# PereUbu7/Variational-Self-Organizing-Maps

Hardware: AMD Instinct MI355X
Metric: training samples/sec per epoch (BMU+update), 128x128 map, 784-dim (higher is better)
Workload: dtype f32

## Files before the change

variational-self-organizing-maps_amd/csrc/vsom_sl_i8.hip:

```cpp
#include "vsom_digits.hpp"
#include <cstdlib>

typedef int v4i __attribute__((ext_vector_type(4)));
typedef int v16i __attribute__((ext_vector_type(16)));
#ifdef VSOM_DEVELOPMENT
__device__ int vsom_sl_dbg = 0;
#endif

__device__ __forceinline__ void sl_kind_mark(unsigned *xflag, unsigned who)
{
    unsigned *slot = xflag + 32 * (1 + (who & 31u));
    if (__atomic_load_n(slot, __ATOMIC_RELAXED) == 0u)
        __atomic_store_n(slot, 1u, __ATOMIC_RELAXED);
}
__device__ __forceinline__ void sl_kind_fold(unsigned *xflag)
{
    const int lane = threadIdx.x & 63;
    const unsigned v = lane < 32 ? xflag[32 * (1 + lane)] : 0u;
    if (__ballot(v != 0u)) {
        if (lane < 32 && v != 0u)
            xflag[32 * (1 + lane)] = 0u;
        if (lane == 0)
            xflag[0] = 1u;
    }
}

__global__ __launch_bounds__(256) void sl_quant_rows_kernel(const float *__restrict__ src, int lds_, float *__restrict__ dst,
                                                            int ldd, const int *__restrict__ idx, int nrows,
                                                            signed char *__restrict__ xi, size_t xplane, int kp8,
                                                            float *__restrict__ lx, size_t lstride, unsigned *__restrict__ xflag)
{
    __shared__ float ssum[4], smax[4], sl1[4], snx[4];
    __shared__ int sa[4];
    const int row = blockIdx.x, lane = threadIdx.x & 63, wave = threadIdx.x >> 6;
    if (row >= nrows)
        return;
    const float *s = src + (size_t)row * lds_;
    auto value = [&](int k) -> float {
        if (k >= ldd)
            return 0.f;
        const int c = idx ? idx[k] : k;
        return c >= 0 ? s[c] : 0.f;
    };
    const int kend = xi ? kp8 : ldd;
    float sum = 0.f, mx = 0.f, l1f = 0.f, nx2 = 0.f;
    bool bad = false;
    float keep[4] = {0.f, 0.f, 0.f, 0.f};
    for (int k4 = threadIdx.x * 4; k4 < kend; k4 += 1024) {
        const float vv[4] = {value(k4), value(k4 + 1), value(k4 + 2), value(k4 + 3)};
#pragma unroll
        for (int u = 0; u < 4; ++u)
            keep[u] = vv[u];
        if (dst && k4 < ldd)
            *reinterpret_cast<float4 *>(dst + (size_t)row * ldd + k4) = make_float4(vv[0], vv[1], vv[2], vv[3]);
// ... 639 lines not shown
__device__ __forceinline__ void sl_gemm_i8_ring_body(const signed char *__restrict__ xi, size_t xplane, int s0, int s1,
                                                     const signed char *__restrict__ q, int N, int kp, int kp8,
                                                     const float *__restrict__ nrm, const double *__restrict__ qscale,
                                                     const double *__restrict__ qcorr, const float *__restrict__ xscale,
                                                     float *__restrict__ G, int ldg, float *__restrict__ tmin, int ntm,
                                                     signed char *ring, const int4 *__restrict__ qfast)
{
    constexpr int AUP = 4 * WM;
    constexpr int AU = AUP * XD;
    constexpr int UNITS = AU + 24;
    constexpr int UPW = UNITS / (2 * WM);
    constexpr int STAGE = UNITS * 1024, QOFF = AU * 1024, RTS = 64 * WM;
    static_assert(UNITS % (2 * WM) == 0 && NS * STAGE <= RING_BYTES, "ring layout");
    const int nchunks = (kp + IK - 1) / IK;
    const int tid = threadIdx.x, lane = tid & 63, wave = tid >> 6;
    const int wm = wave >> 1, wn = wave & 1;
    const int lr = lane & 31, lh = lane >> 5;
    const int sbase = s0 + blockIdx.y * RTS, nbase = blockIdx.x * RT_N;
    const size_t plane = (size_t)N * kp8;
    const signed char *xbase = XD == 1 ? xi : xi + xplane;

    unsigned soff[UPW];
    int dst[UPW];
#pragma unroll
    for (int i = 0; i < UPW; ++i) {
        const int id = wave * UPW + i;
        const int rin = lane >> 2, slot = lane & 3;
        if (id < AU) {
            const int pl = id / AUP, row = (id % AUP) * 16 + rin;
            int sr = sbase + row;
            sr = sr < s1 ? sr : s1 - 1;
            soff[i] = (unsigned)(pl * xplane + (size_t)sr * kp8 + ((slot ^ ((row >> 2) & 3)) << 4));
            dst[i] = id * 1024;
        } else {
            const int pl = (id - AU) >> 3, u = (id - AU) & 7;
            const int row = u * 16 + rin;
            int n = nbase + row;
            n = n < N ? n : N - 1;
            soff[i] = (unsigned)(pl * plane + (size_t)n * kp8 + ((slot ^ ((row >> 2) & 3)) << 4));
            dst[i] = QOFF + pl * 8192 + u * 1024;
        }
    }
    auto issue = [&](int c) {
        const int sb = (c % NS) * STAGE;
#pragma unroll
        for (int i = 0; i < UPW; ++i) {
            const signed char *base = (wave * UPW + i < AU ? xbase : q) + (size_t)c * IK;
            __builtin_amdgcn_global_load_lds((const __attribute__((address_space(1))) void *)(base + soff[i]),
                                             (__attribute__((address_space(3))) void *)(ring + sb + dst[i]), 16, 0, 0);
        }
    };

    v16i acc[3][2][2];
#pragma unroll
    for (int l = 0; l < 3; ++l)
#pragma unroll
        for (int i = 0; i < 2; ++i)
#pragma unroll
            for (int j = 0; j < 2; ++j)
#pragma unroll
                for (int r = 0; r < 16; ++r)
                    acc[l][i][j][r] = 0;

#pragma unroll
    for (int c = 0; c < NS - 1; ++c)
        if (c < nchunks)
            issue(c);
#ifdef VSOM_DEVELOPMENT
    const int dbg = vsom_sl_dbg;
#else
    constexpr int dbg = 0;
#endif
    for (int c = 0; c < ((dbg & 1) ? 1 : nchunks); ++c) {
        if (NS == 3 && c + 1 < nchunks)
            asm volatile("s_waitcnt vmcnt(%0)" ::"n"(UPW) : "memory");
        else
            asm volatile("s_waitcnt vmcnt(0)" ::: "memory");
        __syncthreads();
        if (c + NS - 1 < nchunks)
            issue(c + NS - 1);
        const signed char *st = ring + (c % NS) * STAGE;
#pragma unroll
        for (int ks = 0; ks < 2; ++ks) {
            v4i a[XD][2], b[3][2];
            const int P = ks * 2 + lh;
#pragma unroll
            for (int pl = 0; pl < XD; ++pl)
#pragma unroll
                for (int i = 0; i < 2; ++i) {
                    const int r = wm * 64 + i * 32 + lr;
                    a[pl][i] = *reinterpret_cast<const v4i *>(st + pl * (AUP * 1024) + r * 64 + ((P ^ ((r >> 2) & 3)) << 4));
                }
#pragma unroll
            for (int l = 0; l < 3; ++l)
#pragma unroll
                for (int j = 0; j < 2; ++j) {
                    const int r = wn * 64 + j * 32 + lr;
                    b[l][j] = *reinterpret_cast<const v4i *>(st + QOFF + l * 8192 + r * 64 + ((P ^ ((r >> 2) & 3)) << 4));
                }
#pragma unroll
            for (int pl = 0; pl < XD; ++pl)
#pragma unroll
                for (int l = 0; l + pl < 3; ++l)
#pragma unroll
                    for (int i = 0; i < 2; ++i)
#pragma unroll
                        for (int j = 0; j < 2; ++j)
                            acc[pl + l][i][j] = GLESS
                                                    ? __builtin_amdgcn_mfma_i32_32x32x32_i8(b[l][j], a[pl][i], acc[pl + l][i][j], 0, 0, 0)
                                                    : __builtin_amdgcn_mfma_i32_32x32x32_i8(a[pl][i], b[l][j], acc[pl + l][i][j], 0, 0, 0);
        }
    }
    if (dbg & 2)
        return;
    if (GLESS) {
        float *s_nrm = reinterpret_cast<float *>(ring);
        int4 *s_f = reinterpret_cast<int4 *>(ring + 512);
        __syncthreads();
        if (tid < RT_N) {
            const int n = nbase + tid;
            s_nrm[tid] = n < N ? nrm[n] : __uint_as_float(0x7F800000u);
            s_f[tid] = n < N ? qfast[n] : make_int4(0, 0, 0, 0);
        }
        float ts[2];
        int srow[2];
#pragma unroll
        for (int i = 0; i < 2; ++i) {
            srow[i] = sbase + wm * 64 + i * 32 + lr;
            ts[i] = XD == 3 ? xscale[srow[i] < s1 ? srow[i] : s1 - 1] : 1.f;
        }
        __syncthreads();
#pragma unroll
        for (int j = 0; j < 2; ++j) {
            const int nblk = nbase + wn * 64 + j * 32;
#pragma unroll
            for (int i = 0; i < 2; ++i) {
                float mn = __uint_as_float(0x7F800000u);
#pragma unroll
                for (int r = 0; r < 16; ++r) {
                    const int nl = wn * 64 + j * 32 + 4 * lh + (r & 3) + 8 * (r >> 2);
                    const float g = XD == 1 ? sl_i8_value_fast(acc[0][i][j][r], acc[1][i][j][r], acc[2][i][j][r], s_f[nl], s_nrm[nl])
                                            : sl_i8_value_fast3(acc[0][i][j][r], acc[1][i][j][r], acc[2][i][j][r], s_f[nl], ts[i], s_nrm[nl]);
                    mn = fminf(mn, g);
                }
                if (srow[i] < s1 && nblk < N)
                    tmin[(size_t)(srow[i] - s0) * ntm + (nblk >> 4) + lh] = mn;
            }
        }
        return;
    }
    const float inf = __uint_as_float(0x7F800000u);
    int col[2];
    double nm[2], sc[2], cr[2];
    int4 ff[2];
    float nmf[2];
#pragma unroll
    for (int j = 0; j < 2; ++j) {
        col[j] = nbase + wn * 64 + j * 32 + lr;
        const int cc = col[j] < N ? col[j] : N - 1;
        nmf[j] = nrm[cc];
        if (FAST) {
            ff[j] = qfast[cc];
        } else {
            nm[j] = (double)nmf[j];
            sc[j] = qscale[cc];
            cr[j] = XD == 1 ? qcorr[cc] : 0.0;
        }
    }
#pragma unroll
    for (int i = 0; i < 2; ++i) {
        float rsf[16];
        if (XD != 1) {
#pragma unroll
            for (int r = 0; r < 16; ++r) {
                const int row = sbase + wm * 64 + i * 32 + (r & 3) + 8 * (r >> 2) + 4 * lh;
                rsf[r] = xscale[row < s1 ? row : s1 - 1];
            }
        }
#pragma unroll
        for (int r = 0; r < 16; ++r) {
            float mn = inf;
#pragma unroll
            for (int j = 0; j < 2; ++j) {
                float g;
                if (FAST)
                    g = XD == 1 ? sl_i8_value_fast(acc[0][i][j][r], acc[1][i][j][r], acc[2][i][j][r], ff[j], nmf[j])
                                : sl_i8_value_fast3(acc[0][i][j][r], acc[1][i][j][r], acc[2][i][j][r], ff[j], rsf[r], nmf[j]);
                else
                    g = sl_i8_value(acc[0][i][j][r], acc[1][i][j][r], acc[2][i][j][r], cr[j],
                                    XD == 1 ? sc[j] : sc[j] * (double)rsf[r], nm[j]);
                acc[0][i][j][r] = __float_as_int(g);
                const float m = (col[j] < N && g == g) ? g : inf;
                mn = m < mn ? m : mn;
            }
            acc[1][i][0][r] = __float_as_int(sl_min32_dpp(mn));
        }
    }
    if (dbg & 4)
        return;
#pragma unroll
    for (int i = 0; i < 2; ++i) {
#pragma unroll
        for (int r = 0; r < 16; ++r) {
            const int row = sbase + wm * 64 + i * 32 + (r & 3) + 8 * (r >> 2) + 4 * lh;
            if (row < s1) {
                float *grow = G + (size_t)(row - s0) * ldg;
#pragma unroll
                for (int j = 0; j < 2; ++j)
                    if (col[j] < N)
                        grow[col[j]] = __int_as_float(acc[0][i][j][r]);
                if (lr == 31)
                    tmin[(size_t)(row - s0) * ntm + blockIdx.x * 2 + wn] = __int_as_float(acc[1][i][0][r]);
            }
        }
    }
}

__global__ __launch_bounds__(512, 1) void sl_gemm_i8_ring_kernel(const signed char *__restrict__ xi, size_t xplane, int s0, int s1,
                                                                 const signed char *__restrict__ q, int N, int kp,
                                                                 const unsigned *__restrict__ kp_dev, int kp8,
                                                                 const float *__restrict__ nrm, const double *__restrict__ qscale,
                                                                 const double *__restrict__ qcorr, const float *__restrict__ xscale,
                                                                 float *__restrict__ G, int ldg, float *__restrict__ tmin, int ntm,
                                                                 const unsigned *__restrict__ xflag,
                                                                 const int4 *__restrict__ qfast, unsigned *__restrict__ scal)
{
    if (kp_dev)
        kp = (int)kp_dev[2];
    if (blockIdx.x == 0 && blockIdx.y == 0 && threadIdx.x < 64)
        sl_fold_maxima(scal);
    extern __shared__ __attribute__((aligned(1024))) signed char ring[];
    if (xflag[0] != 0u) {
        if (qfast)
            sl_gemm_i8_ring_body<3, 4, 2, true>(xi, xplane, s0, s1, q, N, kp, kp8, nrm, qscale, qcorr, xscale, G, ldg, tmin, ntm, ring, qfast);
        else
            sl_gemm_i8_ring_body<3, 4, 2, false>(xi, xplane, s0, s1, q, N, kp, kp8, nrm, qscale, qcorr, xscale, G, ldg, tmin, ntm, ring, qfast);
    } else if (qfast)
        sl_gemm_i8_ring_body<1, 4, 3, true>(xi, xplane, s0, s1, q, N, kp, kp8, nrm, qscale, qcorr, xscale, G, ldg, tmin, ntm, ring, qfast);
    else
        sl_gemm_i8_ring_body<1, 4, 3, false>(xi, xplane, s0, s1, q, N, kp, kp8, nrm, qscale, qcorr, xscale, G, ldg, tmin, ntm, ring, qfast);
}

__global__ __launch_bounds__(512, 1) void sl_gemm_i8_ring_gless_kernel(const signed char *__restrict__ xi, size_t xplane, int s0, int s1,
                                                                       const signed char *__restrict__ q, int N, int kp,
                                                                       const unsigned *__restrict__ kp_dev, int kp8,
                                                                       const float *__restrict__ nrm, const float *__restrict__ xscale,
                                                                       float *__restrict__ tmin, int ntl,
                                                                       const unsigned *__restrict__ xflag,
                                                                       const int4 *__restrict__ qfast, unsigned *__restrict__ scal)
{
    if (kp_dev)
        kp = (int)kp_dev[2];
    if (blockIdx.x == 0 && blockIdx.y == 0 && threadIdx.x < 64)
        sl_fold_maxima(scal);
    extern __shared__ __attribute__((aligned(1024))) signed char ring[];
    if (xflag[0] != 0u)
        sl_gemm_i8_ring_body<3, 4, 2, true, true>(xi, xplane, s0, s1, q, N, kp, kp8, nrm, nullptr, nullptr, xscale, nullptr, 0, tmin, ntl, ring, qfast);
    else
        sl_gemm_i8_ring_body<1, 4, 3, true, true>(xi, xplane, s0, s1, q, N, kp, kp8, nrm, nullptr, nullptr, xscale, nullptr, 0, tmin, ntl, ring, qfast);
}

#define K64_NB 16
#define K64_SB 2
template <int XD>
__device__ __forceinline__ void sl_k64_body(const signed char *__restrict__ xi, size_t xplane, int s0, int s1,
                                            const signed char *__restrict__ q, int N, const float *__restrict__ xscale,
                                            float *__restrict__ tmin, int ntl, const float *s_nrm, const int4 *s_f)
{
    const int lane = threadIdx.x & 63, wave = threadIdx.x >> 6;
    const int lr = lane & 31, lh = lane >> 5;
    const int nbase = blockIdx.x * (K64_NB * 32);
    const size_t plane = (size_t)N * 64;
    v4i a[K64_SB][XD][2];
    float ts[K64_SB];
    bool sok[K64_SB];
    float *out[K64_SB];
#pragma unroll
    for (int sb = 0; sb < K64_SB; ++sb) {
        const int srow = s0 + (blockIdx.y * 4 + wave) * (32 * K64_SB) + sb * 32 + lr;
        sok[sb] = srow < s1;
        const size_t sr = (size_t)(sok[sb] ? srow : s1 - 1);
        const signed char *xbase = (XD == 1 ? xi : xi + xplane) + sr * 64 + 16 * lh;
#pragma unroll
        for (int pl = 0; pl < XD; ++pl)
#pragma unroll
            for (int ks = 0; ks < 2; ++ks)
                a[sb][pl][ks] = *reinterpret_cast<const v4i *>(xbase + pl * xplane + ks * 32);
        ts[sb] = XD == 3 ? xscale[sr] : 1.f;
        out[sb] = tmin + (size_t)(srow - s0) * ntl + (nbase >> 4) + lh;
    }
    const int nbn = (N - nbase + 31) / 32 < K64_NB ? (N - nbase + 31) / 32 : K64_NB;
    for (int nb = 0; nb < nbn; ++nb) {
        int n = nbase + nb * 32 + lr;
        n = n < N ? n : N - 1;
        const signed char *qb = q + (size_t)n * 64 + 16 * lh;
        v4i b[3][2];
#pragma unroll
        for (int l = 0; l < 3; ++l)
#pragma unroll
            for (int ks = 0; ks < 2; ++ks)
                b[l][ks] = *reinterpret_cast<const v4i *>(qb + l * plane + ks * 32);
        float nm[16], fx[16];
#pragma unroll
        for (int r = 0; r < 16; ++r) {
            const int nl = nb * 32 + 4 * lh + (r & 3) + 8 * (r >> 2);
            nm[r] = s_nrm[nl];
            fx[r] = __int_as_float(s_f[nl].x);
        }
#pragma unroll
        for (int sb = 0; sb < K64_SB; ++sb) {
            const v16i zero = {0, 0, 0, 0, 0, 0, 0, 0, 0, 0, 0, 0, 0, 0, 0, 0};
            v16i acc[3];
// ... 41 lines not shown
        s_nrm[i] = n < N ? nrm[n] : __uint_as_float(0x7F800000u);
        s_f[i] = n < N ? qfast[n] : make_int4(0, 0, 0, 0);
    }
    if (blockIdx.x == 0 && blockIdx.y == 0 && threadIdx.x < 64)
        sl_fold_maxima(scal);
    __syncthreads();
    if (xflag[0] != 0u)
        sl_k64_body<3>(xi, xplane, s0, s1, q, N, xscale, tmin, ntl, s_nrm, s_f);
    else
        sl_k64_body<1>(xi, xplane, s0, s1, q, N, xscale, tmin, ntl, s_nrm, s_f);
}

static int sl_i8_ensure(vsom_ctx *c, uint32_t kp8)
{
    const bool rekey = !c->sl_q.p || c->sl_kp8 != kp8;
    if (rekey) {
        VSOM_ALLOC_CHECK(vsom_grow_set(c->stream, VSOM_BUF_SYNC | VSOM_BUF_REBUILD,
                                     {vsom_member(c->sl_q, (size_t)3 * c->N * kp8), vsom_member(c->sl_qscale, c->N),
                                      vsom_member(c->sl_qcorr, c->N), vsom_member(c->sl_qfast, c->N)}));
        c->sl_kp8 = kp8;
    }
    if (rekey || (size_t)4 * c->Bcap * kp8 > c->sl_xi.cap) {
        VSOM_ALLOC_CHECK(vsom_grow_set(c->stream, VSOM_BUF_SYNC | VSOM_BUF_REBUILD,
                                     {vsom_member(c->sl_xi, (size_t)4 * c->Bcap * kp8), vsom_member(c->sl_l1, (size_t)5 * c->Bcap)}));
        c->xi_valid = false;
    }
    return VSOM_OK;
}

int launch_sl_gather_quant(vsom_ctx *c, size_t B, hipStream_t stream, const int *idx, bool *xi_out)
{
    const uint32_t kp8 = (c->cpitch + 63) / 64 * 64;
    const bool xi = c->sl_xi.p && c->sl_kp8 == kp8 && (size_t)4 * c->Bcap * kp8 <= c->sl_xi.cap && c->sl_scal.p;
    if (kp8 == 64)
        hipLaunchKernelGGL(sl_quant_rows64_kernel, dim3((unsigned)((B + 15) / 16)), dim3(256), 0, stream, c->Xs.p, (int)c->xpitch, c->Xc.p,
                           (int)c->cpitch, idx, (int)B, xi ? c->sl_xi.p : (signed char *)nullptr, (size_t)c->Bcap * kp8,
                           xi ? c->sl_l1.p : (float *)nullptr, (size_t)c->Bcap, xi ? c->sl_scal.p + 8192 : (unsigned *)nullptr);
    else
    hipLaunchKernelGGL(sl_quant_rows_kernel, dim3((unsigned)B), dim3(256), 0, stream, c->Xs.p, (int)c->xpitch, c->Xc.p,
                       (int)c->cpitch, idx, (int)B, xi ? c->sl_xi.p : (signed char *)nullptr, (size_t)c->Bcap * kp8, (int)kp8,
                       xi ? c->sl_l1.p : (float *)nullptr, (size_t)c->Bcap, xi ? c->sl_scal.p + 8192 : (unsigned *)nullptr);
    VSOM_HIP_CHECK(hipGetLastError());
    *xi_out = xi;
    return VSOM_OK;
}

int sl_i8_plan(vsom_ctx *c, size_t s0, size_t s1)
{
    const uint32_t kp8 = ((c->cc_valid ? c->cpitch : c->xpitch) + 63) / 64 * 64;
    if (kp8 == 64)
        return 1;
    const size_t big_tiles = ((size_t)c->N + RT_N - 1) / RT_N * ((s1 - s0 + RT_S - 1) / RT_S);
    if (kp8 <= 960 && big_tiles >= 256) {
        if (hipFuncSetAttribute((const void *)sl_gemm_i8_ring_gless_kernel, hipFuncAttributeMaxDynamicSharedMemorySize,
                                RING_BYTES) == hipSuccess)
            return 2;
        (void)hipGetLastError();
    }
    return 0;
}

int launch_sl_i8(vsom_ctx *c, size_t s0, size_t s1, size_t ldg, size_t ntm, unsigned *scal, unsigned *xflag, int plan)
{
    const bool gless = plan == 1;
    const bool compact = c->cc_valid;
    const uint32_t kmax = compact ? c->cpitch : c->xpitch;
    const uint32_t kp8 = (kmax + 63) / 64 * 64;
    if (int rc = sl_i8_ensure(c, kp8))
        return rc;
#ifdef VSOM_DEVELOPMENT
    {
        static int last = -1;
        const char *e = std::getenv("VSOM_SL_DBG");
        const int v = e ? std::atoi(e) : 0;
        if (v != last) {
            (void)hipMemcpyToSymbol(HIP_SYMBOL(vsom_sl_dbg), &v, sizeof(int));
            last = v;
        }
    }
#endif
    const size_t xplane = (size_t)c->Bcap * kp8;
    if (!c->xi_valid) {
        if (kp8 == 64)
            hipLaunchKernelGGL(sl_quant_rows64_kernel, dim3((unsigned)((c->B + 15) / 16)), dim3(256), 0, c->stream,
                               compact ? c->Xc.p : c->Xs.p, (int)kmax, (float *)nullptr, (int)kmax, (const int *)nullptr, (int)c->B,
                               c->sl_xi.p, xplane, c->sl_l1.p, (size_t)c->Bcap, xflag);
        else
        hipLaunchKernelGGL(sl_quant_rows_kernel, dim3((unsigned)c->B), dim3(256), 0, c->stream, compact ? c->Xc.p : c->Xs.p, (int)kmax,
                           (float *)nullptr, (int)kmax, (const int *)nullptr, (int)c->B, c->sl_xi.p, xplane, (int)kp8, c->sl_l1.p,
                           (size_t)c->Bcap, xflag);
        c->xi_valid = true;
    }
    const float *xscale = c->sl_l1.p + c->Bcap;
    const unsigned *kp_dev = compact ? (const unsigned *)c->cc_meta.p : nullptr;
    if (kp8 == 64 && c->part_pitch <= 64)
        hipLaunchKernelGGL(sl_prepare64_kernel, dim3((unsigned)((c->N + 15) / 16)), dim3(256), 0, c->stream, c->map.p, (int)c->pitch,
                           (int)c->part_pitch, (int)c->N, compact ? (const int *)c->cc_idx.p : (const int *)nullptr, (int)kmax, kp_dev,
                           c->sl_q.p, c->sl_nrm.p, c->sl_qscale.p, c->sl_qcorr.p, c->sl_qfast.p, scal, xflag);
    else
    hipLaunchKernelGGL(sl_prepare_i8_kernel, dim3((unsigned)((c->N + 3) / 4)), dim3(256), 0, c->stream, c->map.p, (int)c->pitch,
                       (int)c->part_pitch, (int)c->N, compact ? (const int *)c->cc_idx.p : (const int *)nullptr, (int)kmax, kp_dev,
                       (int)kp8, c->sl_q.p, c->sl_nrm.p, c->sl_qscale.p, c->sl_qcorr.p, c->sl_qfast.p, scal, xflag);
    const int4 *qfast = kp8 <= 960 ? c->sl_qfast.p : (const int4 *)nullptr;
    if (gless) {
        if (kp8 != 64)
            return VSOM_ERR_INVALID;
        dim3 grid((unsigned)((c->N + K64_NB * 32 - 1) / (K64_NB * 32)), (unsigned)((s1 - s0 + 128 * K64_SB - 1) / (128 * K64_SB)));
        hipLaunchKernelGGL(sl_k64_kernel, grid, dim3(256), 0, c->stream, c->sl_xi.p, xplane, (int)s0, (int)s1, c->sl_q.p, (int)c->N,
                           c->sl_nrm.p, c->sl_qfast.p, xscale, c->sl_tmin.p, (int)ntm, (const unsigned *)xflag, scal);
        VSOM_HIP_CHECK(hipGetLastError());
        return VSOM_OK;
    }
    if (plan == 2) {
        dim3 grid((unsigned)((c->N + RT_N - 1) / RT_N), (unsigned)((s1 - s0 + RT_S - 1) / RT_S));
        hipLaunchKernelGGL(sl_gemm_i8_ring_gless_kernel, grid, dim3(512), RING_BYTES, c->stream, c->sl_xi.p, xplane, (int)s0, (int)s1,
                           c->sl_q.p, (int)c->N, (int)kmax, kp_dev, (int)kp8, c->sl_nrm.p, xscale, c->sl_tmin.p, (int)ntm,
                           (const unsigned *)xflag, c->sl_qfast.p, scal);
        VSOM_HIP_CHECK(hipGetLastError());
        return VSOM_OK;
    }
    const size_t big_tiles = ((size_t)c->N + RT_N - 1) / RT_N * ((s1 - s0 + RT_S - 1) / RT_S);
    bool ring_ok = false;
    if (big_tiles >= 1024) {
        ring_ok = hipFuncSetAttribute((const void *)sl_gemm_i8_ring_kernel, hipFuncAttributeMaxDynamicSharedMemorySize,
                                      RING_BYTES) == hipSuccess;
        if (!ring_ok)
            (void)hipGetLastError();
    }
    if (ring_ok) {
        dim3 grid((unsigned)(ntm / 2), (unsigned)((s1 - s0 + RT_S - 1) / RT_S));
        hipLaunchKernelGGL(sl_gemm_i8_ring_kernel, grid, dim3(512), RING_BYTES, c->stream, c->sl_xi.p, xplane, (int)s0, (int)s1,
                           c->sl_q.p, (int)c->N, (int)kmax, kp_dev, (int)kp8, c->sl_nrm.p, c->sl_qscale.p, c->sl_qcorr.p, xscale, c->sl_G.p,
                           (int)ldg, c->sl_tmin.p, (int)ntm, (const unsigned *)xflag, qfast, scal);
    } else {
        constexpr int MI = 2;
        dim3 grid((unsigned)ntm, (unsigned)((s1 - s0 + 64 * MI - 1) / (64 * MI)));
        hipLaunchKernelGGL((sl_gemm_i8_kernel<MI, 1>), grid, dim3(256), 0, c->stream, c->sl_xi.p, xplane, (int)s0, (int)s1, c->sl_q.p,
                           (int)c->N, (int)kmax, kp_dev, (int)kp8, c->sl_nrm.p, c->sl_qscale.p, c->sl_qcorr.p, xscale, c->sl_G.p, (int)ldg,
                           c->sl_tmin.p, (int)ntm, (const unsigned *)xflag, qfast, scal);
        hipLaunchKernelGGL((sl_gemm_i8_kernel<MI, 3>), grid, dim3(256), 0, c->stream, c->sl_xi.p, xplane, (int)s0, (int)s1, c->sl_q.p,
                           (int)c->N, (int)kmax, kp_dev, (int)kp8, c->sl_nrm.p, c->sl_qscale.p, c->sl_qcorr.p, xscale, c->sl_G.p, (int)ldg,
                           c->sl_tmin.p, (int)ntm, (const unsigned *)xflag, qfast, scal);
    }
    VSOM_HIP_CHECK(hipGetLastError());
    return VSOM_OK;
}
```

variational-self-organizing-maps_amd/csrc/vsom_update.hip:

```cpp
#include "vsom_device.hpp"
#include <algorithm>
#include <cmath>
#include <cstdlib>
#include <mutex>


#define CWP_WT 512
#define CWP_THREADS (64 + CWP_WT)
template <int NW, int T, bool LUT_LDS, bool CONLY>
__global__ __launch_bounds__(CWP_THREADS) void cwp_kernel(const u64 *__restrict__ lastbmu, int B, int n0, int n1,
                                                          int W, int H, const float *__restrict__ lut,
                                                          int lutw, int luth, float2 *__restrict__ cw, int ldn,
                                                          float *__restrict__ weight)
{
    static_assert(NW * T == 2048 && CWP_WT % NW == 0 && T % 4 == 0 && T <= CWP_WT, "worker mapping");
    constexpr int LK = NW * T / CWP_WT;
    constexpr int PK = LK / 2;
    constexpr int QK = LK / 4;
    static_assert(LK % 4 == 0, "whole sample quads per worker thread");
    constexpr int SS = CWP_WT / NW;
    extern __shared__ __attribute__((aligned(16))) unsigned char cwp_smem[];
    float *wL = (float *)cwp_smem;
    float *WL = wL + 3 * T * NW;
    int2 *bL = (int2 *)(WL + 2 * T * NW);
    float *slut = (float *)(bL + 3 * T);
    const int tid = threadIdx.x;
    if (LUT_LDS) {
        for (int i = tid; i < lutw * luth; i += CWP_THREADS)
            slut[i] = lut[i];
    }
    const float *tab = LUT_LDS ? slut : lut;
    const int ntiles = (B + T - 1) / T;
    const int nloc = n1 - n0;
    const int wt = tid - 64;
    const int lnode = (wt < 0 ? tid : wt) & (NW - 1);
    const int s0 = wt < 0 ? 0 : wt / NW;
    const int nl = blockIdx.x * NW + lnode;
    const bool valid = nl < nloc;
    int cx = 0, cy = 0;
    if (valid)
        vsom_somindex((u64)(n0 + nl), (u64)W, (u64)H, cx, cy);

    auto load_bxy = [&](int t) {
        if (t < ntiles && wt < T) {
            const int j = t * T + wt;
            int bx = 0, by = 0;
            if (j < B)
                vsom_somindex(lastbmu[j], (u64)W, (u64)H, bx, by);
            bL[(t % 3) * T + wt] = make_int2(bx, by);
        }
    };
    auto lookup = [&](int t) {
        float *dst = wL + (t % 3) * T * NW;
        const int2 *bsrc = bL + (t % 3) * T;
        const int nt = B - t * T < T ? B - t * T : T;
        int2 b[LK];
        float w[LK];
#pragma unroll
        for (int k = 0; k < LK; ++k)
            b[k] = bsrc[s0 + k * SS];
#pragma unroll
        for (int k = 0; k < LK; ++k) {
            int dx = cx - b[k].x, dy = cy - b[k].y;
            dx = dx < 0 ? -dx : dx;
            dy = dy < 0 ? -dy : dy;
            dx = dx < lutw ? dx : lutw - 1;
            dy = dy < luth ? dy : luth - 1;
            w[k] = tab[dy * lutw + dx];
        }
#pragma unroll
        for (int k = 0; k < LK; ++k)
            if (s0 + k * SS < nt)
                dst[(s0 + k * SS) * NW + lnode] = w[k];
    };
    auto emit = [&](int t) {
        const float *ws = wL + (t % 3) * T * NW;
        const float *Ws = WL + (t & 1) * T * NW;
        const int nt = B - t * T < T ? B - t * T : T;
        if (CONLY) {
            float w[QK][4], Wp[QK][4];
#pragma unroll
            for (int k = 0; k < QK; ++k) {
                const int s = (s0 + k * SS) * 4;
#pragma unroll
                for (int i = 0; i < 4; ++i) {
                    w[k][i] = ws[(s + i) * NW + lnode];
                    Wp[k][i] = Ws[(s + i) * NW + lnode];
                }
            }
#pragma unroll
            for (int k = 0; k < QK; ++k) {
                const int s = (s0 + k * SS) * 4;
                float4 o;
                o.x = w[k][0] / Wp[k][0];
                o.y = s + 1 < nt ? w[k][1] / Wp[k][1] : 0.f;
                o.z = s + 2 < nt ? w[k][2] / Wp[k][2] : 0.f;
                o.w = s + 3 < nt ? w[k][3] / Wp[k][3] : 0.f;
                if (valid && s < nt)
                    ((float4 *)cw)[(size_t)((t * T + s) >> 2) * ldn + nl] = o;
            }
            return;
        }
        float w0[PK], w1[PK], W0[PK], W1[PK];
#pragma unroll
        for (int k = 0; k < PK; ++k) {
            const int s = (s0 + k * SS) * 2;
            w0[k] = ws[s * NW + lnode];
            W0[k] = Ws[s * NW + lnode];
            w1[k] = ws[(s + 1) * NW + lnode];
            W1[k] = Ws[(s + 1) * NW + lnode];
        }
#pragma unroll
        for (int k = 0; k < PK; ++k) {
            const int s = (s0 + k * SS) * 2;
            float4 o;
            o.x = w0[k] / W0[k];
            o.y = w0[k];
            const bool two = s + 1 < nt;
            o.z = two ? w1[k] / W1[k] : 0.f;
            o.w = two ? w1[k] : 0.f;
            if (valid && s < nt)
                ((float4 *)cw)[(size_t)((t * T + s) >> 1) * ldn + nl] = o;
        }
    };

    float run = 0.f;
    if (wt >= 0) {
        load_bxy(0);
        load_bxy(1);
    }
    __syncthreads();
    if (wt >= 0)
        lookup(0);
    __syncthreads();
    for (int t = 0; t < ntiles; ++t) {
        if (wt >= 0) {
            load_bxy(t + 2);
            if (t + 1 < ntiles)
                lookup(t + 1);
            if (t > 0)
                emit(t - 1);
        } else {
            const float *ws = wL + (t % 3) * T * NW;
            float *Ws = WL + (t & 1) * T * NW;
            const int nt = B - t * T < T ? B - t * T : T;
            int s = 0;
            for (; s + 16 <= nt; s += 16) {
                float r[16], o[16];
#pragma unroll
                for (int k = 0; k < 16; ++k)
                    r[k] = ws[(s + k) * NW + lnode];
#pragma unroll
                for (int k = 0; k < 16; ++k) {
                    run = run + r[k];
                    o[k] = run;
                }
                if (tid < NW) {
#pragma unroll
                    for (int k = 0; k < 16; ++k)
                        Ws[(s + k) * NW + lnode] = o[k];
                }
            }
            for (; s < nt; ++s) {
                run = run + ws[s * NW + lnode];
                if (tid < NW)
                    Ws[s * NW + lnode] = run;
            }
        }
        __syncthreads();
    }
    if (wt >= 0)
        emit(ntiles - 1);
    else if (tid < NW && valid && weight)
        weight[n0 + nl] = run;
}

typedef float vsom_f2 __attribute__((ext_vector_type(2)));

#define VSOM_MED_STEP(XS, CW)                                                                    \
    "v_pk_fma_f32 %[t], %[M], %[k24], " XS " neg_lo:[0,1,0] neg_hi:[0,1,0]\n\t"                   \
    "v_pk_mul_f32 %[p], %[t], %[k127] clamp\n\t"                                                  \
    "v_pk_mul_f32 %[n], %[t], %[k127] neg_lo:[1,0] neg_hi:[1,0] clamp\n\t"                        \
    "v_pk_fma_f32 %[M], " CW ", %[p], %[M] op_sel_hi:[0,1,1]\n\t"                                 \
    "v_pk_fma_f32 %[S], " CW ", %[p], %[S] op_sel:[1,0,0]\n\t"                                    \
    "v_pk_fma_f32 %[M], " CW ", %[n], %[M] op_sel_hi:[0,1,1] neg_lo:[1,0,0] neg_hi:[1,0,0]\n\t"   \
    "v_pk_fma_f32 %[S], " CW ", %[n], %[S] op_sel:[1,0,0]\n\t"

__device__ __forceinline__ void vsom_median_steps8(vsom_f2 &M, vsom_f2 &S, const vsom_f2 (&xs)[8], const float4 (&cv)[4])
{
    const vsom_f2 k24 = {0x1.0p24f, 0x1.0p24f}, k127 = {0x1.0p127f, 0x1.0p127f};
    const vsom_f2 c0 = {cv[0].x, cv[0].y}, c1 = {cv[0].z, cv[0].w}, c2 = {cv[1].x, cv[1].y}, c3 = {cv[1].z, cv[1].w},
                  c4 = {cv[2].x, cv[2].y}, c5 = {cv[2].z, cv[2].w}, c6 = {cv[3].x, cv[3].y}, c7 = {cv[3].z, cv[3].w};
    vsom_f2 t, p, n;
    asm volatile(VSOM_MED_STEP("%[x0]", "%[c0]") VSOM_MED_STEP("%[x1]", "%[c1]") VSOM_MED_STEP("%[x2]", "%[c2]")
                 VSOM_MED_STEP("%[x3]", "%[c3]") VSOM_MED_STEP("%[x4]", "%[c4]") VSOM_MED_STEP("%[x5]", "%[c5]")
                 VSOM_MED_STEP("%[x6]", "%[c6]") VSOM_MED_STEP("%[x7]", "%[c7]")
                 : [M] "+v"(M), [S] "+v"(S), [t] "=&v"(t), [p] "=&v"(p), [n] "=&v"(n)
                 : [x0] "v"(xs[0]), [x1] "v"(xs[1]), [x2] "v"(xs[2]), [x3] "v"(xs[3]), [x4] "v"(xs[4]), [x5] "v"(xs[5]),
                   [x6] "v"(xs[6]), [x7] "v"(xs[7]), [c0] "v"(c0), [c1] "v"(c1), [c2] "v"(c2), [c3] "v"(c3), [c4] "v"(c4),
                   [c5] "v"(c5), [c6] "v"(c6), [c7] "v"(c7), [k24] "s"(k24), [k127] "s"(k127));
}

__device__ __forceinline__ void vsom_median_step1(vsom_f2 &M, vsom_f2 &S, vsom_f2 xs, vsom_f2 cw)
{
    const vsom_f2 k24 = {0x1.0p24f, 0x1.0p24f}, k127 = {0x1.0p127f, 0x1.0p127f};
    vsom_f2 t, p, n;
    asm volatile(VSOM_MED_STEP("%[x0]", "%[c0]")
                 : [M] "+v"(M), [S] "+v"(S), [t] "=&v"(t), [p] "=&v"(p), [n] "=&v"(n)
                 : [x0] "v"(xs), [c0] "v"(cw), [k24] "s"(k24), [k127] "s"(k127));
}

template <bool MEDIAN, int FMA, int PLOG>
__global__ __launch_bounds__(256, 1) void update_chain3_kernel(const float *__restrict__ Xs, int ldx,
                                                               const float2 *__restrict__ cw, int ldn, int B,
                                                               int n0, int nloc, int D,
                                                               float *__restrict__ map,
                                                               float *__restrict__ sigma, int pitch,
                                                               const float *__restrict__ weight)
{
// ... 266 lines not shown
    if (need > c->lut.cap) {
        VSOM_HIP_CHECK(hipStreamSynchronize(c->stream));
        VSOM_ALLOC_CHECK(vsom_grow_set(c->stream, 0, {vsom_member(c->lut, need), vsom_member(c->lut_host, 2 * need)}));
        c->lut_ev_valid[0] = c->lut_ev_valid[1] = false;
    }
    const int k = c->lut_slot;
    c->lut_slot ^= 1;
    if (!c->lut_ev[k])
        VSOM_HIP_CHECK(hipEventCreateWithFlags(&c->lut_ev[k], hipEventDisableTiming));
    if (c->lut_ev_valid[k])
        VSOM_HIP_CHECK(hipEventSynchronize(c->lut_ev[k]));
    float *host = c->lut_host.p + (size_t)k * c->lut.cap;
    for (uint32_t dy = 0; dy < lh; ++dy)
        for (uint32_t dx = 0; dx < lw; ++dx)
            host[(size_t)dy * lw + dx] = (float)vsom_neighbourhood_weight(dx, dy, 0, 0, sigma);
    VSOM_HIP_CHECK(hipMemcpyAsync(c->lut.p, host, need * sizeof(float), hipMemcpyHostToDevice, c->stream));
    VSOM_HIP_CHECK(hipEventRecord(c->lut_ev[k], c->stream));
    c->lut_ev_valid[k] = true;
    c->lut_sigma = sigma;
    c->lut_w = lw;
    c->lut_h = lh;
    return VSOM_OK;
}

__global__ void empty_epoch_kernel(float *__restrict__ map, float *__restrict__ sigma, float *__restrict__ weight,
                                   int pitch, int part_pitch, int part_len, int n0, int nloc)
{
    const size_t i = (size_t)blockIdx.x * blockDim.x + threadIdx.x;
    if (i >= (size_t)nloc * pitch)
        return;
    const int nl = (int)(i / pitch), col = (int)(i % pitch);
    const size_t at = (size_t)(n0 + nl) * pitch + col;
    const float zero = weight[n0 + nl] * 0.f;
    map[at] = 0.f;
    sigma[at] = (col % part_pitch) < part_len ? sqrtf(0.f / (zero * 0.f + 0.f)) : 0.f;
}

__global__ void zero_weight_kernel(float *__restrict__ weight, int n0, int nloc)
{
    const int i = blockIdx.x * blockDim.x + threadIdx.x;
    if (i < nloc)
        weight[n0 + i] = 0.f;
}

static bool vsom_use_chain(const vsom_ctx *c, size_t nloc)
{
    if (!c->use_chain || c->transform == VSOM_CLR)
        return false;
    return ((nloc + 63) / 64) * ((c->D + 13) / 14) <= VSOM_CHAIN_MAX_WAVES;
}

extern "C" int vsom_small_map_chains(const vsom_ctx *c, size_t nodes) { return c && vsom_use_chain(c, nodes) ? 1 : 0; }

static int launch_cwp(vsom_ctx *c, const u64 *bmu, size_t B_, size_t n0, size_t n1, size_t ldn, bool conly, float *weight)
{
    const size_t nloc = n1 - n0;
    const size_t lut_bytes = (size_t)c->lut_w * c->lut_h * sizeof(float);
    const bool lds = lut_bytes <= 24 * 1024;
    constexpr int nw = 16, T = 2048 / nw;
    const size_t smem = (size_t)5 * 2048 * sizeof(float) + (size_t)3 * T * sizeof(int2) + (lds ? lut_bytes : 0);
    const void *fn = conly ? (lds ? (const void *)cwp_kernel<nw, T, true, true> : (const void *)cwp_kernel<nw, T, false, true>)
                           : (lds ? (const void *)cwp_kernel<nw, T, true, false> : (const void *)cwp_kernel<nw, T, false, false>);
    if (smem > 64 * 1024)
        VSOM_HIP_CHECK(hipFuncSetAttribute(fn, hipFuncAttributeMaxDynamicSharedMemorySize, (int)smem));
    int B = (int)B_, in0 = (int)n0, in1 = (int)n1, iW = (int)c->W, iH = (int)c->H, lw = (int)c->lut_w, lh = (int)c->lut_h,
        ildn = (int)ldn;
    const float *lut = c->lut.p;
    float2 *cwp = c->cw.p;
    void *args[] = {&bmu, &B, &in0, &in1, &iW, &iH, &lut, &lw, &lh, &cwp, &ildn, &weight};
    VSOM_HIP_CHECK(hipLaunchKernel(fn, dim3((unsigned)((nloc + nw - 1) / nw)), dim3(CWP_THREADS), args, smem, c->stream));
    return VSOM_OK;
}

static int launch_nt_chains(vsom_ctx *c, void *fn, size_t n0, size_t nloc, size_t B, size_t ldn, uint32_t bpad, bool compact,
                            const unsigned *meta, unsigned block = 512)
{
    const unsigned gx = (unsigned)((nloc + 63) / 64);
    const unsigned cols = compact ? c->cpitch : c->pitch;
    const unsigned quads = compact ? c->cpitch / 4 : (c->D + 3) / 4;
    UpdAsmArgs a;
    a.xs = c->Xq.p;
    a.cw2 = c->cw.p;
    a.map = compact ? c->Uc_map.p : c->map.p;
    a.sbuf = compact ? c->Uc_S.p : c->sigma.p;
    a.ldx_bytes = bpad * 16u;
    a.ldn_bytes = (unsigned)(ldn * 16u);
    a.B = (unsigned)B;
    a.nloc = (unsigned)nloc;
    a.nslices = quads;
    a.pitch_bytes = cols * 4u;
    a.n0 = (unsigned)n0;
    a.ppitch_bytes = 0;
    a.yp = compact ? (const void *)meta : nullptr;
    a.zq = c->zq.p;
    size_t sz = 80;
    void *extra[] = {HIP_LAUNCH_PARAM_BUFFER_POINTER, &a, HIP_LAUNCH_PARAM_BUFFER_SIZE, &sz, HIP_LAUNCH_PARAM_END};
    VSOM_HIP_CHECK(hipModuleLaunchKernel((hipFunction_t)fn, 8 * ((quads + 7) / 8), (gx + 7) / 8, 1, block, 1, 1, 0, c->stream,
                                         nullptr, extra));
    return VSOM_OK;
}

__global__ __launch_bounds__(256) void sg_keep_record_kernel(const int *__restrict__ inv, int ninv, const unsigned *__restrict__ meta,
                                                             int *__restrict__ inv_out, unsigned *__restrict__ meta_out,
                                                             const u64 *__restrict__ bmu, int nb, u64 *__restrict__ bmu_out)
{
    const int i = blockIdx.x * blockDim.x + threadIdx.x;
    if (i < ninv)
        inv_out[i] = inv[i];
    if (i < 16 && ninv > 0)
        meta_out[i] = meta[i];
    if (i < nb)
        bmu_out[i] = bmu[i];
}

void vsom_sigma_drop(vsom_ctx *c)
{
    if (c->sg.on) {
        c->sg.on = false;
        ++c->sg_stats[1];
    }
}

static int sigma_materialise(vsom_ctx *c)
// ... 191 lines not shown
```

Baseline: 1.793 million.

## Specialize gless GEMM by kind and tile size, retune cwp kernel with LDS row swizzle

Templatizes the gless ring GEMM kernel on the x-plane count and wave-M count. It adds a smaller 256-thread, two-blocks-per-CU variant for large grids and launches both kinds, each kernel returning early if the flag does not match. The first chunk's MFMAs now take a zero accumulator instead of an explicit zeroing pass, and the epilogue loads norms and fast coefficients from LDS as vectors. The cwp neighbourhood kernel gains a 112/448 worker configuration with an XOR row rotation meant to cut LDS bank conflicts on large c-only maps. These changes add an extra empty kernel launch and more template instantiations.

```diff
diff --git a/variational-self-organizing-maps_amd/csrc/vsom_sl_i8.hip b/variational-self-organizing-maps_amd/csrc/vsom_sl_i8.hip
--- a/variational-self-organizing-maps_amd/csrc/vsom_sl_i8.hip
+++ b/variational-self-organizing-maps_amd/csrc/vsom_sl_i8.hip
@@ -1,5 +1,6 @@
 #include "vsom_digits.hpp"
 #include <cstdlib>
+#include <type_traits>
 
 typedef int v4i __attribute__((ext_vector_type(4)));
 typedef int v16i __attribute__((ext_vector_type(16)));
@@ -745,15 +746,17 @@
     };
 
     v16i acc[3][2][2];
-#pragma unroll
-    for (int l = 0; l < 3; ++l)
-#pragma unroll
-        for (int i = 0; i < 2; ++i)
-#pragma unroll
-            for (int j = 0; j < 2; ++j)
-#pragma unroll
-                for (int r = 0; r < 16; ++r)
-                    acc[l][i][j][r] = 0;
+    if (!GLESS) {
+#pragma unroll
+        for (int l = 0; l < 3; ++l)
+#pragma unroll
+            for (int i = 0; i < 2; ++i)
+#pragma unroll
+                for (int j = 0; j < 2; ++j)
+#pragma unroll
+                    for (int r = 0; r < 16; ++r)
+                        acc[l][i][j][r] = 0;
+    }
 
 #pragma unroll
     for (int c = 0; c < NS - 1; ++c)
@@ -764,7 +767,8 @@
 #else
     constexpr int dbg = 0;
 #endif
-    for (int c = 0; c < ((dbg & 1) ? 1 : nchunks); ++c) {
+    auto chunk = [&](int c, auto open) {
+        constexpr bool OPEN = decltype(open)::value;
         if (NS == 3 && c + 1 < nchunks)
             asm volatile("s_waitcnt vmcnt(%0)" ::"n"(UPW) : "memory");
         else
@@ -798,11 +802,22 @@
 #pragma unroll
                     for (int i = 0; i < 2; ++i)
 #pragma unroll
-                        for (int j = 0; j < 2; ++j)
+                        for (int j = 0; j < 2; ++j) {
+                            const v16i zero = {0, 0, 0, 0, 0, 0, 0, 0, 0, 0, 0, 0, 0, 0, 0, 0};
+                            const v16i cin = (OPEN && ks == 0 && pl == 0) ? zero : acc[pl + l][i][j];
                             acc[pl + l][i][j] = GLESS
-                                                    ? __builtin_amdgcn_mfma_i32_32x32x32_i8(b[l][j], a[pl][i], acc[pl + l][i][j], 0, 0, 0)
-                                                    : __builtin_amdgcn_mfma_i32_32x32x32_i8(a[pl][i], b[l][j], acc[pl + l][i][j], 0, 0, 0);
-        }
+                                                    ? __builtin_amdgcn_mfma_i32_32x32x32_i8(b[l][j], a[pl][i], cin, 0, 0, 0)
+                                                    : __builtin_amdgcn_mfma_i32_32x32x32_i8(a[pl][i], b[l][j], cin, 0, 0, 0);
+                        }
+        }
+    };
+    if (GLESS) {
+        chunk(0, std::true_type());
+        for (int c = 1; c < ((dbg & 1) ? 1 : nchunks); ++c)
+            chunk(c, std::false_type());
+    } else {
+        for (int c = 0; c < ((dbg & 1) ? 1 : nchunks); ++c)
+            chunk(c, std::false_type());
     }
     if (dbg & 2)
         return;
@@ -823,22 +838,41 @@
             ts[i] = XD == 3 ? xscale[srow[i] < s1 ? srow[i] : s1 - 1] : 1.f;
         }
         __syncthreads();
+        int cb = wn * 64 + 4 * lh;
 #pragma unroll
         for (int j = 0; j < 2; ++j) {
             const int nblk = nbase + wn * 64 + j * 32;
-#pragma unroll
-            for (int i = 0; i < 2; ++i) {
-                float mn = __uint_as_float(0x7F800000u);
-#pragma unroll
-                for (int r = 0; r < 16; ++r) {
-                    const int nl = wn * 64 + j * 32 + 4 * lh + (r & 3) + 8 * (r >> 2);
-                    const float g = XD == 1 ? sl_i8_value_fast(acc[0][i][j][r], acc[1][i][j][r], acc[2][i][j][r], s_f[nl], s_nrm[nl])
-                                            : sl_i8_value_fast3(acc[0][i][j][r], acc[1][i][j][r], acc[2][i][j][r], s_f[nl], ts[i], s_nrm[nl]);
-                    mn = fminf(mn, g);
+            float mn[2] = {__uint_as_float(0x7F800000u), __uint_as_float(0x7F800000u)};
+#pragma unroll
+            for (int h = 0; h < 2; ++h) {
+                const float4 *pn = reinterpret_cast<const float4 *>(s_nrm + cb);
+                const int4 *pf = s_f + cb;
+                float4 nq[2];
+                int4 fq[8];
+#pragma unroll
+                for (int g = 0; g < 2; ++g) {
+                    nq[g] = pn[j * 8 + 4 * h + 2 * g];
+#pragma unroll
+                    for (int k = 0; k < 4; ++k)
+                        fq[4 * g + k] = pf[j * 32 + 16 * h + 8 * g + k];
                 }
+#pragma unroll
+                for (int i = 0; i < 2; ++i)
+#pragma unroll
+                    for (int rr = 0; rr < 8; ++rr) {
+                        const int r = 8 * h + rr;
+                        const float4 n4 = nq[rr >> 2];
+                        const float nm = (rr & 3) == 0 ? n4.x : (rr & 3) == 1 ? n4.y : (rr & 3) == 2 ? n4.z : n4.w;
+                        const float g = XD == 1 ? sl_i8_value_fast(acc[0][i][j][r], acc[1][i][j][r], acc[2][i][j][r], fq[rr], nm)
+                                                : sl_i8_value_fast3(acc[0][i][j][r], acc[1][i][j][r], acc[2][i][j][r], fq[rr], ts[i], nm);
+                        mn[i] = fminf(mn[i], g);
+                    }
+                asm volatile("" : "+v"(mn[0]), "+v"(mn[1]), "+v"(cb));
+            }
+#pragma unroll
+            for (int i = 0; i < 2; ++i)
                 if (srow[i] < s1 && nblk < N)
-                    tmin[(size_t)(srow[i] - s0) * ntm + (nblk >> 4) + lh] = mn;
-            }
+                    tmin[(size_t)(srow[i] - s0) * ntm + (nblk >> 4) + lh] = mn[i];
         }
         return;
     }
@@ -934,7 +968,10 @@
         sl_gemm_i8_ring_body<1, 4, 3, false>(xi, xplane, s0, s1, q, N, kp, kp8, nrm, qscale, qcorr, xscale, G, ldg, tmin, ntm, ring, qfast);
 }
 
-__global__ __launch_bounds__(512, 1) void sl_gemm_i8_ring_gless_kernel(const signed char *__restrict__ xi, size_t xplane, int s0, int s1,
+#define RING_GLESS_NS(XD, WM) ((XD) == 1 && (WM) == 4 ? 3 : 2)
+#define RING_BYTES_GLESS(XD, WM) ((XD) == 3 ? 2 * 73728 : (WM) == 4 ? 3 * 40960 : 2 * 32768)
+template <int XD, int WM>
+__global__ __launch_bounds__(128 * WM, WM == 2 ? 2 : 1) void sl_gemm_i8_ring_gless_kernel(const signed char *__restrict__ xi, size_t xplane, int s0, int s1,
                                                                        const signed char *__restrict__ q, int N, int kp,
                                                                        const unsigned *__restrict__ kp_dev, int kp8,
                                                                        const float *__restrict__ nrm, const float *__restrict__ xscale,
@@ -942,15 +979,16 @@
                                                                        const unsigned *__restrict__ xflag,
                                                                        const int4 *__restrict__ qfast, unsigned *__restrict__ scal)
 {
+    if ((xflag[0] != 0u) != (XD == 3))
+        return;
     if (kp_dev)
         kp = (int)kp_dev[2];
     if (blockIdx.x == 0 && blockIdx.y == 0 && threadIdx.x < 64)
         sl_fold_maxima(scal);
     extern __shared__ __attribute__((aligned(1024))) signed char ring[];
-    if (xflag[0] != 0u)
-        sl_gemm_i8_ring_body<3, 4, 2, true, true>(xi, xplane, s0, s1, q, N, kp, kp8, nrm, nullptr, nullptr, xscale, nullptr, 0, tmin, ntl, ring, qfast);
-    else
-        sl_gemm_i8_ring_body<1, 4, 3, true, true>(xi, xplane, s0, s1, q, N, kp, kp8, nrm, nullptr, nullptr, xscale, nullptr, 0, tmin, ntl, ring, qfast);
+    static_assert(XD == 1 || WM == 4, "general kind: 256 x 128 tiles");
+    sl_gemm_i8_ring_body<XD, WM, RING_GLESS_NS(XD, WM), true, true>(xi, xplane, s0, s1, q, N, kp, kp8, nrm, nullptr, nullptr, xscale, nullptr, 0, tmin,
+                                                              ntl, ring, qfast);
 }
 
 #define K64_NB 16
@@ -1098,8 +1136,12 @@
         return 1;
     const size_t big_tiles = ((size_t)c->N + RT_N - 1) / RT_N * ((s1 - s0 + RT_S - 1) / RT_S);
     if (kp8 <= 960 && big_tiles >= 256) {
-        if (hipFuncSetAttribute((const void *)sl_gemm_i8_ring_gless_kernel, hipFuncAttributeMaxDynamicSharedMemorySize,
-                                RING_BYTES) == hipSuccess)
+        if (hipFuncSetAttribute((const void *)sl_gemm_i8_ring_gless_kernel<1, 4>, hipFuncAttributeMaxDynamicSharedMemorySize,
+                                RING_BYTES_GLESS(1, 4)) == hipSuccess &&
+            hipFuncSetAttribute((const void *)sl_gemm_i8_ring_gless_kernel<1, 2>, hipFuncAttributeMaxDynamicSharedMemorySize,
+                                RING_BYTES_GLESS(1, 2)) == hipSuccess &&
+            hipFuncSetAttribute((const void *)sl_gemm_i8_ring_gless_kernel<3, 4>, hipFuncAttributeMaxDynamicSharedMemorySize,
+                                RING_BYTES_GLESS(3, 4)) == hipSuccess)
             return 2;
         (void)hipGetLastError();
     }
@@ -1159,8 +1201,16 @@
     }
     if (plan == 2) {
         dim3 grid((unsigned)((c->N + RT_N - 1) / RT_N), (unsigned)((s1 - s0 + RT_S - 1) / RT_S));
-        hipLaunchKernelGGL(sl_gemm_i8_ring_gless_kernel, grid, dim3(512), RING_BYTES, c->stream, c->sl_xi.p, xplane, (int)s0, (int)s1,
-                           c->sl_q.p, (int)c->N, (int)kmax, kp_dev, (int)kp8, c->sl_nrm.p, xscale, c->sl_tmin.p, (int)ntm,
+        if ((size_t)grid.x * grid.y >= 1024)
+            hipLaunchKernelGGL((sl_gemm_i8_ring_gless_kernel<1, 2>), dim3(grid.x, (unsigned)((s1 - s0 + 127) / 128)), dim3(256),
+                               RING_BYTES_GLESS(1, 2), c->stream, c->sl_xi.p, xplane, (int)s0, (int)s1, c->sl_q.p, (int)c->N, (int)kmax, kp_dev,
+                               (int)kp8, c->sl_nrm.p, xscale, c->sl_tmin.p, (int)ntm, (const unsigned *)xflag, c->sl_qfast.p, scal);
+        else
+            hipLaunchKernelGGL((sl_gemm_i8_ring_gless_kernel<1, 4>), grid, dim3(512), RING_BYTES_GLESS(1, 4), c->stream, c->sl_xi.p, xplane,
+                               (int)s0, (int)s1, c->sl_q.p, (int)c->N, (int)kmax, kp_dev, (int)kp8, c->sl_nrm.p, xscale, c->sl_tmin.p, (int)ntm,
+                               (const unsigned *)xflag, c->sl_qfast.p, scal);
+        hipLaunchKernelGGL((sl_gemm_i8_ring_gless_kernel<3, 4>), grid, dim3(512), RING_BYTES_GLESS(3, 4), c->stream, c->sl_xi.p, xplane, (int)s0,
+                           (int)s1, c->sl_q.p, (int)c->N, (int)kmax, kp_dev, (int)kp8, c->sl_nrm.p, xscale, c->sl_tmin.p, (int)ntm,
                            (const unsigned *)xflag, c->sl_qfast.p, scal);
         VSOM_HIP_CHECK(hipGetLastError());
         return VSOM_OK;
diff --git a/variational-self-organizing-maps_amd/csrc/vsom_update.hip b/variational-self-organizing-maps_amd/csrc/vsom_update.hip
--- a/variational-self-organizing-maps_amd/csrc/vsom_update.hip
+++ b/variational-self-organizing-maps_amd/csrc/vsom_update.hip
@@ -5,20 +5,26 @@
 #include <mutex>
 
 
-#define CWP_WT 512
-#define CWP_THREADS (64 + CWP_WT)
-template <int NW, int T, bool LUT_LDS, bool CONLY>
-__global__ __launch_bounds__(CWP_THREADS) void cwp_kernel(const u64 *__restrict__ lastbmu, int B, int n0, int n1,
-                                                          int W, int H, const float *__restrict__ lut,
-                                                          int lutw, int luth, float2 *__restrict__ cw, int ldn,
-                                                          float *__restrict__ weight)
-{
-    static_assert(NW * T == 2048 && CWP_WT % NW == 0 && T % 4 == 0 && T <= CWP_WT, "worker mapping");
-    constexpr int LK = NW * T / CWP_WT;
+template <int NW, bool ROT>
+__device__ __forceinline__ int cwp_row(int s)
+{
+    return ROT ? (s * NW) ^ (((s >> 2) & 1) << 4) : s * NW;
+}
+
+template <int NW, int T, int WT, bool LUT_LDS, bool CONLY, bool ROT>
+__global__ __launch_bounds__(64 + WT) void cwp_kernel(const u64 *__restrict__ lastbmu, int B, int n0, int n1,
+                                                      int W, int H, const float *__restrict__ lut,
+                                                      int lutw, int luth, float2 *__restrict__ cw, int ldn,
+                                                      float *__restrict__ weight)
+{
+    constexpr int CWP_THREADS = 64 + WT;
+    static_assert((NW * T) % WT == 0 && WT % NW == 0 && T % 16 == 0 && T <= WT, "worker mapping");
+    static_assert(!ROT || (NW == 16 && CONLY), "the rotation is that of the c-only emit over 16-float rows");
+    constexpr int LK = NW * T / WT;
     constexpr int PK = LK / 2;
     constexpr int QK = LK / 4;
     static_assert(LK % 4 == 0, "whole sample quads per worker thread");
-    constexpr int SS = CWP_WT / NW;
+    constexpr int SS = WT / NW;
     extern __shared__ __attribute__((aligned(16))) unsigned char cwp_smem[];
     float *wL = (float *)cwp_smem;
     float *WL = wL + 3 * T * NW;
@@ -71,7 +77,7 @@
 #pragma unroll
         for (int k = 0; k < LK; ++k)
             if (s0 + k * SS < nt)
-                dst[(s0 + k * SS) * NW + lnode] = w[k];
+                dst[cwp_row<NW, ROT>(s0 + k * SS) + lnode] = w[k];
     };
     auto emit = [&](int t) {
         const float *ws = wL + (t % 3) * T * NW;
@@ -84,8 +90,8 @@
                 const int s = (s0 + k * SS) * 4;
 #pragma unroll
                 for (int i = 0; i < 4; ++i) {
-                    w[k][i] = ws[(s + i) * NW + lnode];
-                    Wp[k][i] = Ws[(s + i) * NW + lnode];
+                    w[k][i] = ws[cwp_row<NW, ROT>(s + i) + lnode];
+                    Wp[k][i] = Ws[cwp_row<NW, ROT>(s + i) + lnode];
                 }
             }
 #pragma unroll
@@ -149,7 +155,7 @@
                 float r[16], o[16];
 #pragma unroll
                 for (int k = 0; k < 16; ++k)
-                    r[k] = ws[(s + k) * NW + lnode];
+                    r[k] = ws[s * NW + lnode + cwp_row<NW, ROT>(k)];
 #pragma unroll
                 for (int k = 0; k < 16; ++k) {
                     run = run + r[k];
@@ -158,13 +164,13 @@
                 if (tid < NW) {
 #pragma unroll
                     for (int k = 0; k < 16; ++k)
-                        Ws[(s + k) * NW + lnode] = o[k];
+                        Ws[s * NW + lnode + cwp_row<NW, ROT>(k)] = o[k];
                 }
             }
             for (; s < nt; ++s) {
-                run = run + ws[s * NW + lnode];
+                run = run + ws[cwp_row<NW, ROT>(s) + lnode];
                 if (tid < NW)
-                    Ws[s * NW + lnode] = run;
+                    Ws[cwp_row<NW, ROT>(s) + lnode] = run;
             }
         }
         __syncthreads();
@@ -537,15 +543,29 @@
 
 extern "C" int vsom_small_map_chains(const vsom_ctx *c, size_t nodes) { return c && vsom_use_chain(c, nodes) ? 1 : 0; }
 
+template <int T, int WT, bool ROT>
+static const void *cwp_fn(bool lds, bool conly)
+{
+    if (conly)
+        return lds ? (const void *)cwp_kernel<16, T, WT, true, true, ROT> : (const void *)cwp_kernel<16, T, WT, false, true, ROT>;
+    return lds ? (const void *)cwp_kernel<16, T, WT, true, false, false> : (const void *)cwp_kernel<16, T, WT, false, false, false>;
+}
+
 static int launch_cwp(vsom_ctx *c, const u64 *bmu, size_t B_, size_t n0, size_t n1, size_t ldn, bool conly, float *weight)
 {
     const size_t nloc = n1 - n0;
     const size_t lut_bytes = (size_t)c->lut_w * c->lut_h * sizeof(float);
     const bool lds = lut_bytes <= 24 * 1024;
-    constexpr int nw = 16, T = 2048 / nw;
-    const size_t smem = (size_t)5 * 2048 * sizeof(float) + (size_t)3 * T * sizeof(int2) + (lds ? lut_bytes : 0);
-    const void *fn = conly ? (lds ? (const void *)cwp_kernel<nw, T, true, true> : (const void *)cwp_kernel<nw, T, false, true>)
-                           : (lds ? (const void *)cwp_kernel<nw, T, true, false> : (const void *)cwp_kernel<nw, T, false, false>);
+    constexpr int nw = 16;
+    const size_t nwg = (nloc + nw - 1) / nw;
+    bool four = conly && nwg > 3 * 256;
+#ifdef VSOM_DEVELOPMENT
+    if (std::getenv("VSOM_CWP_T128"))
+        four = false;
+#endif
+    const int T = four ? 112 : 128, WT = four ? 448 : 512;
+    const void *fn = four ? cwp_fn<112, 448, true>(lds, true) : cwp_fn<128, 512, false>(lds, conly);
+    const size_t smem = (size_t)5 * nw * T * sizeof(float) + (size_t)3 * T * sizeof(int2) + (lds ? lut_bytes : 0);
     if (smem > 64 * 1024)
         VSOM_HIP_CHECK(hipFuncSetAttribute(fn, hipFuncAttributeMaxDynamicSharedMemorySize, (int)smem));
     int B = (int)B_, in0 = (int)n0, in1 = (int)n1, iW = (int)c->W, iH = (int)c->H, lw = (int)c->lut_w, lh = (int)c->lut_h,
@@ -553,7 +573,7 @@
     const float *lut = c->lut.p;
     float2 *cwp = c->cw.p;
     void *args[] = {&bmu, &B, &in0, &in1, &iW, &iH, &lut, &lw, &lh, &cwp, &ildn, &weight};
-    VSOM_HIP_CHECK(hipLaunchKernel(fn, dim3((unsigned)((nloc + nw - 1) / nw)), dim3(CWP_THREADS), args, smem, c->stream));
+    VSOM_HIP_CHECK(hipLaunchKernel(fn, dim3((unsigned)nwg), dim3(64 + WT), args, smem, c->stream));
     return VSOM_OK;
 }
 
```

After: 1.772 million. -1.2%, worse.
